# fboehm/DBSLMM

Hardware: AMD Instinct MI355X
Metric: SNPs solved/sec (whole node) + max-|Δβ| vs CPU ref, 1M SNP × 10k indiv (higher is better)
Workload: dtype f64

## Files before the change

### dbslmm_amd/csrc/pcg.hip

```cpp
#include <hip/hip_runtime.h>
#include <stdint.h>

namespace pcg {
constexpr int kT = 128;
constexpr int kRunMax = 8;
constexpr int kMaxNC = 4;
constexpr int kWaves = 4;
constexpr int kVS = kT + 8;
constexpr int kNDot = 5;
constexpr int kQS = 8;
constexpr int kThreads = 256;
constexpr int kFTb = 8;
constexpr int kFRows = kFTb * kT;
constexpr int kFPer = kFRows / kThreads;
constexpr int wave_lds_doubles(int nc) { return 3 * nc * kVS + 4 * nc * 64; }
constexpr size_t lds_bytes(int nc) { return sizeof(double) * kWaves * wave_lds_doubles(nc); }
}

struct PcgBlk {
    int32_t blk, row0, m, ms;
    int32_t ld, Tb, Ns, sco;
    int64_t matoff, vo, po, dof;
    int64_t off16;
    int32_t nc;
    int32_t mshift;
    int32_t fused;
    int32_t pad_;
};

struct PcgArgs {
    const PcgBlk* blk;
    const uint16_t* G16;
    const double* M;
    const int32_t* flags;
    const double* S;
    const double* rsd;
    const double* z;
    const int32_t* slot_out;
    const int32_t* blk_id;
    const double* dshift;
    double *X, *R, *P, *Sv, *W;
    double* U;
    double* part;
    double* dot;
    double* qs;
    int32_t* cnv;
    int32_t* itb;
    int32_t* done;
    int32_t* active;
    int32_t* fin;
    double* beta_s;
    double* beta_l;
    int32_t* status;
    double* mir_s;
    double* mir_l;
    int32_t* mir_st;
    int32_t* mir_flag;
    int32_t run_no;
    int64_t vstride;
    int64_t ns, nl, nbk;
    double tau, rn, c0, tol, inv_sqrt_n;
    int32_t ncopy;
    int32_t run;
    int32_t seed;
};

namespace pcg {

__device__ __forceinline__ void wave_fence() {
    __builtin_amdgcn_fence(__ATOMIC_RELEASE, "wavefront");
    __builtin_amdgcn_wave_barrier();
    __builtin_amdgcn_fence(__ATOMIC_ACQUIRE, "wavefront");
}

template <int Ctrl>
__device__ __forceinline__ double dpp_mov(double v) {
    const uint64_t b = __builtin_bit_cast(uint64_t, v);
    const int lo = __builtin_amdgcn_mov_dpp(static_cast<int>(b & 0xffffffffu), Ctrl, 0xf, 0xf, false);
    const int hi = __builtin_amdgcn_mov_dpp(static_cast<int>(b >> 32), Ctrl, 0xf, 0xf, false);
    return __builtin_bit_cast(double, (static_cast<uint64_t>(static_cast<uint32_t>(hi)) << 32) | static_cast<uint32_t>(lo));
}
template <int X>
__device__ __forceinline__ uint32_t swap_xor(uint32_t x, bool up) {
    if constexpr (X == 16) {
        const auto r = __builtin_amdgcn_permlane16_swap(x, x, false, false);
        return up ? r[0] : r[1];
    } else {
        const auto r = __builtin_amdgcn_permlane32_swap(x, x, false, false);
        return up ? r[0] : r[1];
    }
}
template <int X>
__device__ __forceinline__ double lane_xor(double v) {
#ifndef PCG_NO_DPP
    if constexpr (X == 1) return dpp_mov<0xB1>(v);
    else if constexpr (X == 2) return dpp_mov<0x4E>(v);
    else if constexpr (X == 4) return dpp_mov<0x1B>(dpp_mov<0x141>(v));
    else if constexpr (X == 8) return dpp_mov<0x128>(v);
#ifndef PCG_NO_PERMLANE
    else if constexpr (X == 16 || X == 32) {
        const uint64_t b = __builtin_bit_cast(uint64_t, v);
        const bool up = (__lane_id() & X) != 0;
        const uint32_t lo = swap_xor<X>(static_cast<uint32_t>(b & 0xffffffffu), up);
        const uint32_t hi = swap_xor<X>(static_cast<uint32_t>(b >> 32), up);
        return __builtin_bit_cast(double, (static_cast<uint64_t>(hi) << 32) | lo);
    }
#endif
    else
#endif
        return __shfl_xor(v, X);
}

template <int X2, int X1, int X0>
__device__ __forceinline__ double rscatter8(const double (&v)[8], int lane) {
    const bool h2 = (lane & X2) != 0, h1 = (lane & X1) != 0, h0 = (lane & X0) != 0;
    double u[4], w[2];
#pragma unroll
    for (int q = 0; q < 4; ++q) {
        const double send = h2 ? v[q] : v[q + 4], keep = h2 ? v[q + 4] : v[q];
        u[q] = keep + lane_xor<X2>(send);
    }
#pragma unroll
    for (int q = 0; q < 2; ++q) {
        const double send = h1 ? u[q] : u[q + 2], keep = h1 ? u[q + 2] : u[q];
        w[q] = keep + lane_xor<X1>(send);
    }
    const double send = h0 ? w[0] : w[1], keep = h0 ? w[1] : w[0];
    return keep + lane_xor<X0>(send);
}

__device__ __forceinline__ double wave_sum(double v) {
    v += lane_xor<32>(v);
    v += lane_xor<16>(v);
    v += lane_xor<8>(v);
    v += lane_xor<4>(v);
    v += lane_xor<2>(v);
    v += lane_xor<1>(v);
    return v;
}



__device__ __forceinline__ double ordered_sum(const double* __restrict__ p, int64_t st, int s0, int s1, double acc) {
    for (int s = s0; s < s1; s += 8) {
        double t[8];
#pragma unroll
        for (int u = 0; u < 8; ++u) t[u] = s + u < s1 ? p[static_cast<int64_t>(s + u) * st] : 0.0;
#pragma unroll
        for (int u = 0; u < 8; ++u) acc += t[u];
    }
    return acc;
}

__device__ __forceinline__ bool on_u16(const PcgArgs& a, const PcgBlk& B) {
    return a.G16 != nullptr && (a.flags[B.blk] & 1) == 0;
}

__device__ __forceinline__ double jdiag(const PcgArgs& a, const PcgBlk& B, int i, double dc) {
    return B.mshift ? 1.0 : i < B.ms ? a.c0 + dc : a.c0;
}
__device__ __forceinline__ double col_shift(const PcgArgs& a, const PcgBlk& B, int k) {
    return a.dshift[B.mshift ? a.seed : k];
}

__device__ __forceinline__ void put_beta(const PcgArgs& a, const PcgBlk& B, int i, int k, double x, bool mono) {
    const int so = a.slot_out[B.row0 + i];
    const double bv = mono ? __builtin_nan("") : x * a.inv_sqrt_n;
    if (so >= 0) {
        a.beta_s[k * a.ns + so] = bv;
        if (a.mir_s) a.mir_s[k * a.ns + so] = bv;
    } else {
        a.beta_l[k * a.nl - 1 - so] = bv;
        if (a.mir_l) a.mir_l[k * a.nl - 1 - so] = bv;
    }
}
__device__ __forceinline__ void put_status(const PcgArgs& a, const PcgBlk& B, int k, bool mono) {
    const int st = mono ? DBSLMM_BLOCK_MONOMORPHIC
                        : a.cnv[B.sco + k] == 0 ? DBSLMM_BLOCK_NOT_CONVERGED : DBSLMM_BLOCK_OK;
    const int64_t o = k * a.nbk + a.blk_id[B.blk];
    a.status[o] = st;
    if (a.mir_st) a.mir_st[o] = st;
}

__device__ __forceinline__ double cvt_lo(uint32_t w) {
    double g;
    uint32_t t;
    asm volatile("v_and_b32 %1, 0xffff, %2\n\tv_cvt_f64_u32 %0, %1" : "=v"(g), "=&v"(t) : "v"(w));
    return g;
}
__device__ __forceinline__ double cvt_hi(uint32_t w) {
    double g;
    uint32_t t;
    asm volatile("v_lshrrev_b32 %1, 16, %2\n\tv_cvt_f64_u32 %0, %1" : "=v"(g), "=&v"(t) : "v"(w));
    return g;
}

typedef uint32_t pcg_u4 __attribute__((ext_vector_type(4)));

__device__ __forceinline__ __amdgpu_buffer_rsrc_t g16_rsrc(const uint16_t* base, uint32_t bytes) {
    const uint64_t gb = reinterpret_cast<uint64_t>(base);
    const uint32_t lo = static_cast<uint32_t>(__builtin_amdgcn_readfirstlane(static_cast<int>(gb & 0xffffffffu)));
    const uint32_t hi = static_cast<uint32_t>(__builtin_amdgcn_readfirstlane(static_cast<int>(gb >> 32)));
    const int nb = __builtin_amdgcn_readfirstlane(static_cast<int>(bytes));
    return __builtin_amdgcn_make_buffer_rsrc(reinterpret_cast<void*>((static_cast<uint64_t>(hi) << 32) | lo),
                                             static_cast<short>(0), nb, 0x00020000);
}
constexpr uint32_t kG16Oob = 0x80000000u;

__device__ __forceinline__ void quad_mul16(const pcg_u4 (&raw)[8], bool diagq, int lane, int nc,
                                           const double* vI, const double* vJ, double* rsum, double* csum) {
    const int rg = lane >> 3, cg = lane & 7;
#pragma unroll 1
    for (int k = 0; k < nc; ++k) {
        double vi[8], vj[8], racc[8], cacc[8];
#pragma unroll
        for (int q = 0; q < 8; ++q) {
            vi[q] = vI[k * kVS + 8 * rg + q];
            vj[q] = vJ[k * kVS + 8 * cg + q];
            racc[q] = cacc[q] = 0.0;
        }
        if (!diagq) {
#pragma unroll
            for (int r = 0; r < 8; ++r)
#pragma unroll
                for (int c = 0; c < 8; ++c) {
                    const uint32_t w = raw[r][c >> 1];
                    const double g = (c & 1) ? cvt_hi(w) : cvt_lo(w);
                    racc[r] = __builtin_fma(g, vj[c], racc[r]);
                    cacc[c] = __builtin_fma(g, vi[r], cacc[c]);
                }
        } else {
#pragma unroll
            for (int r = 0; r < 8; ++r)
#pragma unroll
                for (int c = 0; c < 8; ++c) {
                    const uint32_t w = raw[r][c >> 1];
                    const double g = (c & 1) ? cvt_hi(w) : cvt_lo(w);
                    const int dd = 8 * (cg - rg) + c - r;
                    racc[r] = __builtin_fma(dd <= 0 ? g : 0.0, vj[c], racc[r]);
                    cacc[c] = __builtin_fma(dd < 0 ? g : 0.0, vi[r], cacc[c]);
                }
        }
        rsum[k * 64 + lane] += rscatter8<4, 2, 1>(racc, lane);
        csum[k * 64 + lane] += rscatter8<32, 16, 8>(cacc, lane);
    }
}

__device__ __forceinline__ void quad_mul64(const double* __restrict__ base, int64_t ld, int rows_ok, int cols_ok,
                                           bool diagq, int lane, int nc, const double* vI, const double* vJ,
                                           double* rsum, double* csum) {
    const int rg = lane >> 3, cg = lane & 7;
#pragma unroll 1
    for (int k = 0; k < nc; ++k) {
        double vi[8], vj[8], racc[8], cacc[8];
#pragma unroll
        for (int q = 0; q < 8; ++q) {
            vi[q] = vI[k * kVS + 8 * rg + q];
            vj[q] = vJ[k * kVS + 8 * cg + q];
            racc[q] = cacc[q] = 0.0;
        }
#pragma unroll 1
        for (int r = 0; r < 8; ++r)
#pragma unroll
            for (int c = 0; c < 8; ++c) {
                const double g = (r < rows_ok && c < cols_ok) ? base[r * ld + c] : 0.0;
                const int dd = 8 * (cg - rg) + c - r;
                const double gr = !diagq || dd <= 0 ? g : 0.0, gc = !diagq || dd < 0 ? g : 0.0;
#pragma unroll
                for (int q = 0; q < 8; ++q)
                    if (q == r) racc[q] = __builtin_fma(gr, vj[c], racc[q]);
                cacc[c] = __builtin_fma(gc, vi[r], cacc[c]);
            }
        rsum[k * 64 + lane] += rscatter8<4, 2, 1>(racc, lane);
        csum[k * 64 + lane] += rscatter8<32, 16, 8>(cacc, lane);
    }
}

__device__ __forceinline__ void stage_v(const PcgArgs& a, const PcgBlk& B, int T, int nc, int lane, double* v) {
    for (int k = 0; k < nc; ++k) {
        const double* src = a.U + k * a.vstride + B.vo + static_cast<int64_t>(T) * kT;
        const double x0 = src[lane], x1 = src[lane + 64];
        v[k * kVS + lane] = x0;
        v[k * kVS + lane + 64] = x1;
    }
}

__device__ __forceinline__ bool quad_active(const PcgBlk& B, int I, int J, int q) {
    const int qi = q >> 1, qj = q & 1;
    return !(J == I && qj > qi) && I * kT + 64 * qi < B.m && J * kT + 64 * qj < B.m;
}
__device__ __forceinline__ bool next_quad(const PcgBlk& B, int I, int J1, int& J, int& q) {
    for (;;) {
        if (++q == 4) {
            q = 0;
            if (++J > J1) return false;
        }
        if (quad_active(B, I, J, q)) return true;
    }
}

template <bool U16>
__device__ void symv_item(const PcgArgs& a, int4 item, int lane, double* vI, double* vJb, double* rsum,
                          double* csum) {
    const PcgBlk B = a.blk[item.x];
    if (a.done[item.x] || on_u16(a, B) != U16) return;
    const int I = item.y, J0 = item.z, J1 = item.w, nc = B.nc;
    const int64_t ld16 = static_cast<int64_t>(B.Tb) * kT;
    const int rg = lane >> 3, cg = lane & 7;
    auto vj_of = [&](int J) -> double* { return J == I ? vI : vJb + ((J - J0) & 1) * nc * kVS; };
    const __amdgpu_buffer_rsrc_t g16 =
        g16_rsrc(a.G16 + B.off16 + static_cast<int64_t>(I) * kT * ld16, U16 ? static_cast<uint32_t>(kT * ld16 * 2) : 0u);
    auto load = [&](int J, int q, pcg_u4 (&raw)[8], bool none) {
        if constexpr (U16) {
            const int i0 = 64 * (q >> 1) + 8 * rg, j0 = J * kT + 64 * (q & 1) + 8 * cg;
            const bool skip = none || j0 >= B.m || (J == I && (q == 0 || q == 3) && cg > rg);
            const uint32_t o = static_cast<uint32_t>((static_cast<int64_t>(i0) * ld16 + j0) * 2);
#pragma unroll
            for (int r = 0; r < 8; ++r)
                raw[r] = __builtin_amdgcn_raw_buffer_load_b128(
                    g16, (skip || I * kT + i0 + r >= B.m) ? kG16Oob : o + static_cast<uint32_t>(r * ld16 * 2), 0, 0);
        }
    };
    auto mult = [&](int J, int q, const pcg_u4 (&raw)[8]) {
        const int qi = q >> 1, qj = q & 1;
        const bool dq = J == I && qi == qj;
        const double* vj = vj_of(J);
        double* rs = rsum + qi * nc * 64;
        double* cs = csum + qj * nc * 64;
        if constexpr (U16) {
            quad_mul16(raw, dq, lane, nc, vI + 64 * qi, vj + 64 * qj, rs, cs);
        } else {
            const int ib = I * kT + 64 * qi + 8 * rg, jb = J * kT + 64 * qj + 8 * cg;
            quad_mul64(a.M + B.matoff + static_cast<int64_t>(ib) * B.ld + jb, B.ld, B.m - ib, B.m - jb, dq,
                       lane, nc, vI + 64 * qi, vj + 64 * qj, rs, cs);
        }
    };
    auto flush = [&](int J) {
        double* dst = a.part + B.po + (static_cast<int64_t>(J) * B.Ns + I) * nc * kT;
        for (int qj = 0; qj < 2; ++qj)
            for (int k = 0; k < nc; ++k) {
                dst[k * kT + 64 * qj + 8 * cg + rg] = csum[(qj * nc + k) * 64 + lane];
                csum[(qj * nc + k) * 64 + lane] = 0.0;
            }
    };
    pcg_u4 ra[8], rb[8];
    int J = J0, q = 0;
    load(J, q, ra, false);
    stage_v(a, B, I, nc, lane, vI);
    if (J != I) stage_v(a, B, J, nc, lane, vj_of(J));
    for (int t = 0; t < 2 * nc; ++t) rsum[t * 64 + lane] = csum[t * 64 + lane] = 0.0;
    wave_fence();
    auto step = [&](pcg_u4 (&cur)[8], pcg_u4 (&nxt)[8]) -> bool {
        int Jn = J, qn = q;
        const bool more = next_quad(B, I, J1, Jn, qn);
        load(more ? Jn : J, more ? qn : q, nxt, !more);
        if (more && Jn != J && Jn != I) stage_v(a, B, Jn, nc, lane, vj_of(Jn));
        mult(J, q, cur);
        if (!more || Jn != J) flush(J);
        wave_fence();
        J = Jn;
        q = qn;
        return more;
    };
    while (step(ra, rb) && step(rb, ra)) {
    }
    double* dst = a.part + B.po + (static_cast<int64_t>(I) * B.Ns + B.Tb + J0 / a.run) * nc * kT;
    for (int qi = 0; qi < 2; ++qi)
        for (int k = 0; k < nc; ++k) dst[k * kT + 64 * qi + 8 * rg + cg] = rsum[(qi * nc + k) * 64 + lane];
}

}

extern "C" __global__ __launch_bounds__(pcg::kThreads) void dbslmm_pcg_init(PcgArgs a, const int2* __restrict__ rows) {
    using namespace pcg;
    __shared__ double red[kThreads / 64][kMaxNC];
    __shared__ int mono_s;
    const int2 it = rows[blockIdx.x];
    const int bi = it.x, I = it.y, tid = threadIdx.x;
    const PcgBlk B = a.blk[bi];
    const bool u16 = on_u16(a, B);
    const int n = a.ncopy, nc = B.nc;
    if (I == 0) {
        if (tid == 0) mono_s = 0;
        __syncthreads();
        bool mono = false;
        for (int i = tid; i < B.m; i += kThreads) mono |= !(a.rsd[B.row0 + i] < INFINITY);
        if (mono) atomicOr(&mono_s, 1);
        __syncthreads();
        if (tid < n) {
            a.cnv[B.sco + tid] = 0;
            double* q = a.qs + static_cast<int64_t>(B.sco + tid) * kQS;
            q[4] = q[5] = 1.0;
        }
        if (tid == 0) {
            a.itb[bi] = 0;
            a.fin[bi] = 0;
            const bool fz = B.fused && u16;
            a.done[bi] = mono_s ? 2 : fz ? 3 : 0;
            if (!mono_s && !fz) atomicAdd(a.active, 1);
        }
    }
    const int r = tid & (kT - 1), h = tid >> 7, i = I * kT + r;
    const bool in = i < B.m;
    double sv[kMaxNC];
#pragma unroll
    for (int k = 0; k < kMaxNC; ++k) sv[k] = 0.0;
    for (int c = h; c < n; c += 2) {
        const int64_t o = c * a.vstride + B.vo + i;
        const double rhs = in ? a.z[B.row0 + i] : 0.0;
        a.X[o] = 0.0;
        a.P[o] = 0.0;
        if (c < nc) {
            a.Sv[o] = 0.0;
            a.W[o] = 0.0;
            a.R[o] = rhs;
            double uv = 0.0;
            if (in) {
                uv = rhs / jdiag(a, B, i, col_shift(a, B, c));
                if (u16) uv *= a.rsd[B.row0 + i];
            }
            a.U[o] = uv;
        }
    }
#pragma unroll
    for (int k = 0; k < kMaxNC; ++k)
        if (k < nc && (k & 1) == h && in && u16) {
            const double rhs = a.z[B.row0 + i];
            sv[k] = a.S[B.row0 + i] * a.rsd[B.row0 + i] * (rhs / jdiag(a, B, i, col_shift(a, B, k)));
        }
#pragma unroll
    for (int k = 0; k < kMaxNC; ++k) sv[k] = wave_sum(sv[k]);
    if ((tid & 63) == 0)
#pragma unroll
        for (int k = 0; k < kMaxNC; ++k) red[tid >> 6][k] = sv[k];
    __syncthreads();
    if (tid < nc) {
        const int hk = tid & 1;
        a.dot[B.dof + (static_cast<int64_t>(I) * kNDot + 4) * n + tid] = red[2 * hk][tid] + red[2 * hk + 1][tid];
    }
}

template <bool U16>
__device__ __forceinline__ void symv_body(const PcgArgs& a, const int4* __restrict__ items, int32_t n_items) {
    using namespace pcg;
    extern __shared__ double vlds[];
    const int wave = threadIdx.x >> 6, lane = threadIdx.x & 63;
    const int e = blockIdx.x * kWaves + wave;
    if (e >= n_items) return;
    const int nc = a.ncopy;
    double* w = vlds + wave * wave_lds_doubles(nc);
    symv_item<U16>(a, items[e], lane, w, w + nc * kVS, w + 3 * nc * kVS, w + 3 * nc * kVS + 2 * nc * 64);
}
#ifndef PCG_SYMV_WAVES
#define PCG_SYMV_WAVES 2
#endif
extern "C" __global__ __launch_bounds__(pcg::kThreads) __attribute__((amdgpu_waves_per_eu(PCG_SYMV_WAVES, 8)))
void dbslmm_pcg_symv16(PcgArgs a, const int4* __restrict__ items, int32_t n_items) {
    symv_body<true>(a, items, n_items);
}
extern "C" __global__ __launch_bounds__(pcg::kThreads)
void dbslmm_pcg_symv64(PcgArgs a, const int4* __restrict__ items, int32_t n_items) {
    symv_body<false>(a, items, n_items);
}

extern "C" __global__ __launch_bounds__(pcg::kThreads) void dbslmm_pcg_rows(PcgArgs a, const int2* __restrict__ rows) {
    using namespace pcg;
    __shared__ double red[kThreads / 64][kMaxNC][4];
    __shared__ double sig[kMaxNC];
    const int2 it = rows[blockIdx.x];
    const int bi = it.x, I = it.y, tid = threadIdx.x;
    if (a.done[bi]) return;
    const PcgBlk B = a.blk[bi];
    const bool u16 = on_u16(a, B);
    const int n = a.ncopy, nc = B.nc;
    if (tid < nc)
        sig[tid] = ordered_sum(a.dot + B.dof + 4 * n + tid, kNDot * n, 0, B.Tb, 0.0);
    __syncthreads();
    const int r = tid & (kT - 1), h = tid >> 7, i = I * kT + r;
    const bool in = i < B.m;
    const double Si = in ? a.S[B.row0 + i] : 0.0, ri = in ? a.rsd[B.row0 + i] : 0.0;
    const int nrun = (I + a.run) / a.run;
    double dv[kMaxNC][4];
#pragma unroll
    for (int k = 0; k < kMaxNC; ++k)
#pragma unroll
        for (int f = 0; f < 4; ++f) dv[k][f] = 0.0;
#pragma unroll
    for (int k = 0; k < kMaxNC; ++k) {
        if (k >= n || (k & 1) != h) continue;
        const int64_t o = k * a.vstride + B.vo + i;
        if (k < nc) {
            const double* pp = a.part + B.po + static_cast<int64_t>(I) * B.Ns * nc * kT + k * kT + r;
            double y = ordered_sum(pp, nc * kT, I, B.Tb, 0.0);
            y = ordered_sum(pp, nc * kT, B.Tb, B.Tb + nrun, y);
            const double dc = col_shift(a, B, k);
            const double rv = a.R[o];
            const double u = in ? rv / jdiag(a, B, i, dc) : 0.0;
            const double sh = i < B.ms ? dc : 0.0;
            double w = 0.0;
            if (in) {
                if (u16) w = a.tau * a.rn * ri * __builtin_fma(-Si, sig[k] * a.rn, y) + (1.0 - a.tau + sh) * u;
                else w = y + sh * u;
            }
            a.W[o] = w;
            dv[k][0] = rv * u;
            dv[k][1] = w * u;
            dv[k][2] = rv * rv;
        }
        const double xv = a.X[o];
        dv[k][3] = xv * xv;
    }
#pragma unroll
    for (int k = 0; k < kMaxNC; ++k)
#pragma unroll
        for (int f = 0; f < 4; ++f) dv[k][f] = wave_sum(dv[k][f]);
    if ((tid & 63) == 0)
#pragma unroll
        for (int k = 0; k < kMaxNC; ++k)
#pragma unroll
            for (int f = 0; f < 4; ++f) red[tid >> 6][k][f] = dv[k][f];
    __syncthreads();
    if (tid < 4 * n) {
        const int k = tid >> 2, f = tid & 3, hk = k & 1;
        if (f == 3 || k < nc)
            a.dot[B.dof + (static_cast<int64_t>(I) * kNDot + f) * n + k] = red[2 * hk][k][f] + red[2 * hk + 1][k][f];
    }
    if (I == 0 && tid == 0) a.itb[bi] += 1;
}

extern "C" __global__ __launch_bounds__(pcg::kThreads) void dbslmm_pcg_update(PcgArgs a, const int2* __restrict__ rows) {
    using namespace pcg;
    __shared__ double tot[kMaxNC][4];
    __shared__ double coef[kMaxNC][3];
    __shared__ double seedc[2];
    __shared__ int run_s[kMaxNC];
    __shared__ double red[kThreads / 64][kMaxNC];
    const int2 it = rows[blockIdx.x];
    const int bi = it.x, I = it.y, tid = threadIdx.x;
    if (a.done[bi]) return;
    const PcgBlk B = a.blk[bi];
    const bool u16 = on_u16(a, B);
    const int n = a.ncopy, nc = B.nc;
    const int itn = a.itb[bi] - 1;
    const int par = itn & 1;
    if (tid < 4 * n) {
        const int k = tid >> 2, f = tid & 3;
        tot[k][f] = (f == 3 || k < nc) ? ordered_sum(a.dot + B.dof + f * n + k, kNDot * n, 0, B.Tb, 0.0) : 0.0;
    }
    __syncthreads();
    if (B.mshift) {
        if (tid == 0) {
            const double gam = tot[0][0], del = tot[0][1];
            const double* q = a.qs + static_cast<int64_t>(B.sco) * kQS;
            double al, be = 0.0;
            if (itn == 0) {
                al = gam / del;
            } else {
                be = gam / q[2 * par];
                al = gam / (del - be * gam / q[2 * par + 1]);
            }
            seedc[0] = al;
            seedc[1] = be;
        }
        __syncthreads();
        if (tid < n) {
            const int c = tid;
            double* q = a.qs + static_cast<int64_t>(B.sco + c) * kQS;
            const double al = seedc[0], be = seedc[1];
            const double zk = q[4 + 2 * par], zk1 = q[4 + 2 * par + 1];
            const double rr = tot[0][2] * zk * zk, xx = tot[c][3];
            const double t = a.tol * (a.dshift[c] + 1.0 - a.tau);
            const bool conv = a.cnv[B.sco + c] != 0 || rr == 0.0 || rr <= t * t * xx;
            const double e = a.dshift[c] - a.dshift[a.seed];
            const double cp = itn == 0 ? 0.0 : al * be / a.qs[static_cast<int64_t>(B.sco) * kQS + 2 * par + 1];
            const double zn = zk * zk1 / ((1.0 + cp + al * e) * zk1 - cp * zk);
            coef[c][0] = al * zn / zk;
            coef[c][1] = zk1 != 0.0 ? (zk / zk1) * (zk / zk1) * be : 0.0;
            coef[c][2] = zk;
            run_s[c] = conv ? 0 : 1;
            if (I == 0) {
                if (conv && a.cnv[B.sco + c] == 0) a.cnv[B.sco + c] = itn + 1;
                q[4 + 2 * (par ^ 1)] = zn;
                q[4 + 2 * (par ^ 1) + 1] = zk;
            }
        }
        __syncthreads();
        if (I == 0 && tid == 0) {
            double* q = a.qs + static_cast<int64_t>(B.sco) * kQS;
            q[2 * (par ^ 1)] = tot[0][0];
            q[2 * (par ^ 1) + 1] = seedc[0];
        }
    } else {
        if (tid < n) {
            const int k = tid;
            const double gam = tot[k][0], del = tot[k][1], rr = tot[k][2], xx = tot[k][3];
            const double lam = B.ms == B.m ? a.dshift[k] + 1.0 - a.tau : 1.0 - a.tau;
            const double t = a.tol * lam;
            const bool conv = a.cnv[B.sco + k] != 0 || rr == 0.0 || rr <= t * t * xx;
            double al = 0.0, be = 0.0;
            if (!conv) {
                double* q = a.qs + static_cast<int64_t>(B.sco + k) * kQS;
                if (itn == 0) {
                    al = gam / del;
                } else {
                    be = gam / q[2 * par];
                    al = gam / (del - be * gam / q[2 * par + 1]);
                }
                if (I == 0) {
                    q[2 * (par ^ 1)] = gam;
                    q[2 * (par ^ 1) + 1] = al;
                }
            } else if (I == 0 && a.cnv[B.sco + k] == 0) {
                a.cnv[B.sco + k] = itn + 1;
            }
            coef[k][0] = al;
            coef[k][1] = be;
            coef[k][2] = 1.0;
            run_s[k] = conv ? 0 : 1;
        }
        __syncthreads();
    }
    int running = 0;
    for (int k = 0; k < n; ++k) running += run_s[k];
    if (running == 0) {
        const int r = tid & (kT - 1), h = tid >> 7, i = I * kT + r;
        if (i < B.m)
            for (int k = h; k < n; k += 2) put_beta(a, B, i, k, a.X[k * a.vstride + B.vo + i], false);
        if (I == 0 && tid < n) put_status(a, B, tid, false);
        __syncthreads();
        if (tid == 0 &&
            __hip_atomic_fetch_add(a.fin + bi, 1, __ATOMIC_ACQ_REL, __HIP_MEMORY_SCOPE_AGENT) == B.Tb - 1) {
            a.done[bi] = 1;
            atomicSub(a.active, 1);
            if (a.mir_flag)
                for (int c = 0; c < n; ++c)
                    __hip_atomic_store(a.mir_flag + static_cast<int64_t>(bi) * n + c, a.run_no, __ATOMIC_RELEASE,
                                       __HIP_MEMORY_SCOPE_SYSTEM);
        }
        return;
    }
    const int r = tid & (kT - 1), h = tid >> 7, i = I * kT + r;
    const bool in = i < B.m;
    double sv[kMaxNC];
#pragma unroll
    for (int k = 0; k < kMaxNC; ++k) sv[k] = 0.0;
    if (B.mshift) {
        if (in) {
            const int64_t o0 = B.vo + i;
            const double rv = a.R[o0];
#pragma unroll
            for (int c = 0; c < kMaxNC; ++c) {
                if (c >= n || (c & 1) != h || !run_s[c]) continue;
                const int64_t o = c * a.vstride + o0;
                const double p = __builtin_fma(coef[c][1], a.P[o], coef[c][2] * rv);
                a.P[o] = p;
                a.X[o] = __builtin_fma(coef[c][0], p, a.X[o]);
            }
            if (h == 0) {
                const double al = seedc[0], be = seedc[1];
                const double sn = __builtin_fma(be, a.Sv[o0], a.W[o0]);
                const double rn = __builtin_fma(-al, sn, rv);
                a.Sv[o0] = sn;
                a.R[o0] = rn;
                a.U[o0] = u16 ? rn * a.rsd[B.row0 + i] : rn;
                if (u16) sv[0] = a.S[B.row0 + i] * a.rsd[B.row0 + i] * rn;
            }
        }
    } else {
#pragma unroll
        for (int k = 0; k < kMaxNC; ++k) {
            if (k >= n || (k & 1) != h || !run_s[k] || !in) continue;
            const int64_t o = k * a.vstride + B.vo + i;
            const double al = coef[k][0], be = coef[k][1];
            const double dg = jdiag(a, B, i, a.dshift[k]);
            const double u = a.R[o] / dg;
            const double p = __builtin_fma(be, a.P[o], u);
            const double s = __builtin_fma(be, a.Sv[o], a.W[o]);
            const double x = __builtin_fma(al, p, a.X[o]);
            const double rn = __builtin_fma(-al, s, a.R[o]);
            a.P[o] = p;
            a.Sv[o] = s;
            a.X[o] = x;
            a.R[o] = rn;
            a.U[o] = u16 ? (rn / dg) * a.rsd[B.row0 + i] : rn / dg;
            if (u16) sv[k] = a.S[B.row0 + i] * a.rsd[B.row0 + i] * (rn / dg);
        }
    }
#pragma unroll
    for (int k = 0; k < kMaxNC; ++k) sv[k] = wave_sum(sv[k]);
    if ((tid & 63) == 0)
#pragma unroll
        for (int k = 0; k < kMaxNC; ++k) red[tid >> 6][k] = sv[k];
    __syncthreads();
    if (tid < nc && (B.mshift || run_s[tid])) {
        const int hk = tid & 1;
        a.dot[B.dof + (static_cast<int64_t>(I) * kNDot + 4) * n + tid] = red[2 * hk][tid] + red[2 * hk + 1][tid];
    }
}

#ifndef PCG_BLOCK_DEPTH
#define PCG_BLOCK_DEPTH 3
#endif
namespace pcg {
template <int N>
__device__ __forceinline__ void block_sum(double (&v)[N], double* red, int tid) {
#pragma unroll
    for (int k = 0; k < N; ++k) v[k] = wave_sum(v[k]);
    __syncthreads();
    if ((tid & 63) == 0)
#pragma unroll
        for (int k = 0; k < N; ++k) red[(tid >> 6) * N + k] = v[k];
    __syncthreads();
#pragma unroll
    for (int k = 0; k < N; ++k) v[k] = ((red[k] + red[N + k]) + red[2 * N + k]) + red[3 * N + k];
}
constexpr size_t block_lds_bytes(int n) {
    return sizeof(double) * ((5 + 2 * n) * kFRows + 4 * (3 + kMaxNC) + 12 + 3 * kMaxNC + 4);
}
}

__device__ __forceinline__ void pcg_block_solve(const PcgArgs& a, int bi, int cc, int32_t maxit) {
    using namespace pcg;
    extern __shared__ double blds[];
    double* yw = blds;
    double* Ul = blds + 4 * kFRows;
    const int n = a.ncopy;
    double* Xl = Ul + kFRows;
    double* Pl = Xl + n * kFRows;
    double* red = Pl + n * kFRows;
    if (a.done[bi] != 3) return;
    const PcgBlk B = a.blk[bi];
    const int tid = threadIdx.x, lane = tid & 63, wave = tid >> 6;
    const int m = B.m, Tb = B.Tb;
    const bool msh = cc < 0;
    const int nx = msh ? n : 1;
    const double dc = msh ? col_shift(a, B, 0) : a.dshift[cc];
    double r[kFPer], sv[kFPer], wv[kFPer], Sr[kFPer], Rr[kFPer], sg[1] = {0.0};
#pragma unroll
    for (int q = 0; q < kFPer; ++q) {
        const int i = tid + kThreads * q;
        const bool in = i < m;
        r[q] = in ? a.z[B.row0 + i] : 0.0;
        Sr[q] = in ? a.S[B.row0 + i] : 0.0;
        Rr[q] = in ? a.rsd[B.row0 + i] : 0.0;
        sv[q] = wv[q] = 0.0;
        double u = 0.0;
        if (in) {
            u = (r[q] / jdiag(a, B, i, dc)) * Rr[q];
            sg[0] += Sr[q] * u;
        }
        Ul[i] = u;
        for (int w = 0; w < 4; ++w) yw[w * kFRows + i] = 0.0;
        for (int c = 0; c < nx; ++c) Xl[c * kFRows + i] = Pl[c * kFRows + i] = 0.0;
    }
    block_sum(sg, red, tid);
    double sig = sg[0];
    const int Q = (m + 63) / 64;
    const int nq = Q * (Q + 1) / 2;
    const int64_t ld16 = static_cast<int64_t>(Tb) * kT;
    const int rg = lane >> 3, cg = lane & 7;
    auto quad_of = [&](int t, int& qi, int& qj) {
        qi = static_cast<int>((sqrtf(8.0f * t + 1.0f) - 1.0f) * 0.5f);
        while (qi * (qi + 1) / 2 > t) --qi;
        while ((qi + 1) * (qi + 2) / 2 <= t) ++qi;
        qj = t - qi * (qi + 1) / 2;
    };
    const __amdgpu_buffer_rsrc_t g16 = g16_rsrc(a.G16 + B.off16, static_cast<uint32_t>(ld16 * ld16 * 2));
    auto load = [&](int t, pcg_u4 (&raw)[8]) {
        int qi, qj;
        quad_of(t, qi, qj);
        const int r0 = 64 * qi + 8 * rg, c0 = 64 * qj + 8 * cg;
        const bool skip = t >= nq || c0 >= m || (qi == qj && cg > rg);
        const uint32_t o = static_cast<uint32_t>((r0 * static_cast<int>(ld16) + c0) * 2);
#pragma unroll
        for (int rr = 0; rr < 8; ++rr)
            raw[rr] = __builtin_amdgcn_raw_buffer_load_b128(
                g16, (skip || r0 + rr >= m) ? kG16Oob : o + static_cast<uint32_t>(rr * ld16 * 2), 0, 0);
    };
    auto mult = [&](int t, const pcg_u4 (&raw)[8]) {
        int qi, qj;
        quad_of(t, qi, qj);
        const bool dq = qi == qj;
        double vi[8], vj[8], racc[8], cacc[8];
#pragma unroll
        for (int q = 0; q < 8; ++q) {
            vi[q] = Ul[64 * qi + 8 * rg + q];
            vj[q] = Ul[64 * qj + 8 * cg + q];
            racc[q] = cacc[q] = 0.0;
        }
        if (!dq) {
#pragma unroll
            for (int rr = 0; rr < 8; ++rr)
#pragma unroll
                for (int c = 0; c < 8; ++c) {
                    const uint32_t w = raw[rr][c >> 1];
                    const double g = (c & 1) ? cvt_hi(w) : cvt_lo(w);
                    racc[rr] = __builtin_fma(g, vj[c], racc[rr]);
                    cacc[c] = __builtin_fma(g, vi[rr], cacc[c]);
                }
        } else {
#pragma unroll
            for (int rr = 0; rr < 8; ++rr)
#pragma unroll
                for (int c = 0; c < 8; ++c) {
                    const uint32_t w = raw[rr][c >> 1];
                    const double g = (c & 1) ? cvt_hi(w) : cvt_lo(w);
                    const int dd = 8 * (cg - rg) + c - rr;
                    racc[rr] = __builtin_fma(dd <= 0 ? g : 0.0, vj[c], racc[rr]);
                    cacc[c] = __builtin_fma(dd < 0 ? g : 0.0, vi[rr], cacc[c]);
                }
        }
        double* y = yw + wave * kFRows;
        const int ri = 64 * qi + 8 * rg + cg, ci = 64 * qj + 8 * cg + rg;
        y[ri] += rscatter8<4, 2, 1>(racc, lane);
        wave_fence();
        y[ci] += rscatter8<32, 16, 8>(cacc, lane);
    };
    double* st = red + 4 * (3 + kMaxNC);
    int* flag = reinterpret_cast<int*>(st + 12 + 3 * kMaxNC);
    if (tid == 0) {
        for (int c = 0; c < kMaxNC; ++c) {
            st[4 + c] = st[8 + c] = 1.0;
            flag[c] = c >= n;
        }
    }
    int it = 0;
    for (; it < maxit; ++it) {
        __syncthreads();
        {
#if PCG_BLOCK_DEPTH == 3
            pcg_u4 ra[8], rb[8], rc[8];
            int t = wave;
            load(t, ra);
            load(t + 4, rb);
            while (t < nq) {
                load(t + 8, rc);
                mult(t, ra);
                t += 4;
                if (t >= nq) break;
                load(t + 8, ra);
                mult(t, rb);
                t += 4;
                if (t >= nq) break;
                load(t + 8, rb);
                mult(t, rc);
                t += 4;
            }
#else
            pcg_u4 ra[8], rb[8];
            int t = wave;
            load(t, ra);
            while (t < nq) {
                load(t + 4, rb);
                mult(t, ra);
                t += 4;
                if (t >= nq) break;
                load(t + 4, ra);
                mult(t, rb);
                t += 4;
            }
#endif
        }
        __syncthreads();
        double d[3 + kMaxNC];
#pragma unroll
        for (int k = 0; k < 3 + kMaxNC; ++k) d[k] = 0.0;
#pragma unroll
        for (int q = 0; q < kFPer; ++q) {
            const int i = tid + kThreads * q;
            double y = 0.0;
            if (i < Tb * kT) {
                y = ((yw[i] + yw[kFRows + i]) + yw[2 * kFRows + i]) + yw[3 * kFRows + i];
#pragma unroll
                for (int w = 0; w < 4; ++w) yw[w * kFRows + i] = 0.0;
            }
            if (i < m) {
                const double Si = Sr[q], ri = Rr[q];
                const double u = r[q] / jdiag(a, B, i, dc);
                const double sh = i < B.ms ? dc : 0.0;
                const double w = a.tau * a.rn * ri * __builtin_fma(-Si, sig * a.rn, y) + (1.0 - a.tau + sh) * u;
                wv[q] = w;
                d[0] += r[q] * u;
                d[1] += w * u;
                d[2] += r[q] * r[q];
                for (int c = 0; c < nx; ++c) {
                    const double xv = Xl[c * kFRows + i];
                    d[3 + c] += xv * xv;
                }
            }
        }
        block_sum(d, red, tid);
        if (tid == 0) {
            const double gam = d[0], del = d[1], rr = d[2];
            double al, be = 0.0;
            if (it == 0) {
                al = gam / del;
            } else {
                be = gam / st[0];
                al = gam / (del - be * gam / st[1]);
            }
            int running = 0;
            if (msh) {
                const double cp = it == 0 ? 0.0 : al * be / st[1];
                for (int c = 0; c < n; ++c) {
                    const double zk = st[4 + c], zk1 = st[8 + c];
                    const double t = a.tol * (a.dshift[c] + 1.0 - a.tau);
                    const double rrc = rr * zk * zk;
                    if (!flag[c] && (rrc == 0.0 || rrc <= t * t * d[3 + c])) {
                        flag[c] = 1;
                        a.cnv[B.sco + c] = it + 1;
                    }
                    const double e = a.dshift[c] - a.dshift[a.seed];
                    const double zn = zk * zk1 / ((1.0 + cp + al * e) * zk1 - cp * zk);
                    st[12 + 3 * c] = al * zn / zk;
                    st[12 + 3 * c + 1] = zk1 != 0.0 ? (zk / zk1) * (zk / zk1) * be : 0.0;
                    st[12 + 3 * c + 2] = zk;
                    st[8 + c] = zk;
                    st[4 + c] = zn;
                    running += flag[c] ? 0 : 1;
                }
            } else {
                const double lam = B.ms == B.m ? dc + 1.0 - a.tau : 1.0 - a.tau;
                const double t = a.tol * lam;
                if (rr == 0.0 || rr <= t * t * d[3]) {
                    flag[0] = 1;
                    a.cnv[B.sco + cc] = it + 1;
                }
                running = flag[0] ? 0 : 1;
            }
            st[0] = gam;
            st[1] = al;
            st[2] = al;
            st[3] = be;
            flag[kMaxNC] = running;
        }
        __syncthreads();
        if (flag[kMaxNC] == 0) break;
        const double al = st[2], be = st[3];
        double sg2[1] = {0.0};
#pragma unroll
        for (int q = 0; q < kFPer; ++q) {
            const int i = tid + kThreads * q;
            if (i >= m) continue;
            const double rsd_i = Rr[q];
            double rn;
            if (msh) {
                for (int c = 0; c < n; ++c) {
                    if (flag[c]) continue;
                    const int o = c * kFRows + i;
                    const double pv = __builtin_fma(st[12 + 3 * c + 1], Pl[o], st[12 + 3 * c + 2] * r[q]);
                    Pl[o] = pv;
                    Xl[o] = __builtin_fma(st[12 + 3 * c], pv, Xl[o]);
                }
                const double sn = __builtin_fma(be, sv[q], wv[q]);
                rn = __builtin_fma(-al, sn, r[q]);
                sv[q] = sn;
                r[q] = rn;
                Ul[i] = rn * rsd_i;
            } else {
                const double dg = jdiag(a, B, i, dc);
                const double u = r[q] / dg;
                const double pv = __builtin_fma(be, Pl[i], u);
                const double sn = __builtin_fma(be, sv[q], wv[q]);
                Pl[i] = pv;
                Xl[i] = __builtin_fma(al, pv, Xl[i]);
                rn = __builtin_fma(-al, sn, r[q]);
                sv[q] = sn;
                r[q] = rn;
                Ul[i] = (rn / dg) * rsd_i;
            }
            sg2[0] += Sr[q] * Ul[i];
        }
        block_sum(sg2, red, tid);
        sig = sg2[0];
    }
#pragma unroll
    for (int q = 0; q < kFPer; ++q) {
        const int i = tid + kThreads * q;
        if (i < m)
            for (int c = 0; c < nx; ++c) put_beta(a, B, i, msh ? c : cc, Xl[c * kFRows + i], false);
    }
    if (tid == 0) {
        atomicMax(a.itb + bi, it + (it < maxit ? 1 : 0));
        for (int c = 0; c < nx; ++c) put_status(a, B, msh ? c : cc, false);
    }
    if (a.mir_flag) {
        __syncthreads();
        if (tid == 0)
            for (int c = 0; c < nx; ++c)
                __hip_atomic_store(a.mir_flag + static_cast<int64_t>(bi) * n + (msh ? c : cc), a.run_no,
                                   __ATOMIC_RELEASE, __HIP_MEMORY_SCOPE_SYSTEM);
    }
}

extern "C" __global__ __launch_bounds__(pcg::kThreads)
#if PCG_BLOCK_DEPTH == 3
__attribute__((amdgpu_waves_per_eu(1, 8), amdgpu_num_vgpr(312)))
#else
__attribute__((amdgpu_waves_per_eu(2, 8)))
#endif
void dbslmm_pcg_block(PcgArgs a, const int2* __restrict__ list, int32_t n_list, int32_t* __restrict__ next,
                      int32_t maxit) {
    __shared__ int e_s;
    for (;;) {
        __syncthreads();
        if (threadIdx.x == 0) e_s = atomicAdd(next, 1);
        __syncthreads();
        const int e = e_s;
        if (e >= n_list) break;
        pcg_block_solve(a, list[e].x, list[e].y, maxit);
    }
}

extern "C" __global__ __launch_bounds__(pcg::kThreads) void dbslmm_pcg_final(PcgArgs a, const int2* __restrict__ rows) {
    using namespace pcg;
    const int2 it = rows[blockIdx.x];
    const int bi = it.x, I = it.y, tid = threadIdx.x;
    const int done = a.done[bi];
    if (done == 3 || done == 1) return;
    const PcgBlk B = a.blk[bi];
    const bool mono = done == 2;
    const int r = tid & (kT - 1), h = tid >> 7, i = I * kT + r;
    if (i < B.m)
        for (int k = h; k < a.ncopy; k += 2) put_beta(a, B, i, k, a.X[k * a.vstride + B.vo + i], mono);
    if (I == 0 && tid < a.ncopy) put_status(a, B, tid, mono);
}
```

Measured before the change: 156.5 million.

## Hoist global loads ahead of reductions and widen ordered-sum batches in PCG kernels

The rows and update kernels now issue their per-element loads (R, X, P, Sv, W, S, rsd, partial sums) up front, before the barrier and the cross-tile dot reductions, so load latency overlaps the serial reductions. Lanes at the end of the block now compute the sigma reduction instead of the first lanes. The ordered_sum helper moves to a shared header with a templated batch width of 16 instead of 8, and the partial-sum loop is merged into one call. The block solve preloads slot_out and block id and takes status from a local convergence flag instead of re-reading global memory. The cost is higher register pressure, plus reliance on a `flag` variable that must exist in the elided code.

New measurement: 158.9 million, median of 4. 1.02x the previous value.

```diff
diff --git a/dbslmm_amd/csrc/ordered_sum.hpp b/dbslmm_amd/csrc/ordered_sum.hpp
--- /dev/null
+++ b/dbslmm_amd/csrc/ordered_sum.hpp
@@ -0,0 +1,26 @@
+#pragma once
+#include <stdint.h>
+
+#if defined(__HIPCC__)
+#define ORDERED_SUM_FN __attribute__((host)) __attribute__((device)) inline __attribute__((always_inline))
+#else
+#define ORDERED_SUM_FN inline
+#endif
+#if defined(__clang__)
+#define ORDERED_SUM_UNROLL _Pragma("unroll")
+#else
+#define ORDERED_SUM_UNROLL
+#endif
+
+template <int B = 32>
+ORDERED_SUM_FN double ordered_sum(const double* __restrict__ p, int64_t st, int s0, int s1, double acc) {
+    static_assert(B > 0, "batch width");
+    for (int s = s0; s < s1; s += B) {
+        double t[B];
+        ORDERED_SUM_UNROLL
+        for (int u = 0; u < B; ++u) t[u] = s + u < s1 ? p[static_cast<int64_t>(s + u) * st] : 0.0;
+        ORDERED_SUM_UNROLL
+        for (int u = 0; u < B; ++u) acc += t[u];
+    }
+    return acc;
+}
diff --git a/dbslmm_amd/csrc/pcg.hip b/dbslmm_amd/csrc/pcg.hip
--- a/dbslmm_amd/csrc/pcg.hip
+++ b/dbslmm_amd/csrc/pcg.hip
@@ -1,5 +1,7 @@
 #include <hip/hip_runtime.h>
 #include <stdint.h>
+
+#include "ordered_sum.hpp"
 
 namespace pcg {
 constexpr int kT = 128;
@@ -10,6 +12,7 @@
 constexpr int kNDot = 5;
 constexpr int kQS = 8;
 constexpr int kThreads = 256;
+constexpr int kSumBatch = 16;
 constexpr int kFTb = 8;
 constexpr int kFRows = kFTb * kT;
 constexpr int kFPer = kFRows / kThreads;
@@ -139,19 +142,6 @@
     return v;
 }
 
-
-
-__device__ __forceinline__ double ordered_sum(const double* __restrict__ p, int64_t st, int s0, int s1, double acc) {
-    for (int s = s0; s < s1; s += 8) {
-        double t[8];
-#pragma unroll
-        for (int u = 0; u < 8; ++u) t[u] = s + u < s1 ? p[static_cast<int64_t>(s + u) * st] : 0.0;
-#pragma unroll
-        for (int u = 0; u < 8; ++u) acc += t[u];
-    }
-    return acc;
-}
-
 __device__ __forceinline__ bool on_u16(const PcgArgs& a, const PcgBlk& B) {
     return a.G16 != nullptr && (a.flags[B.blk] & 1) == 0;
 }
@@ -163,8 +153,7 @@
     return a.dshift[B.mshift ? a.seed : k];
 }
 
-__device__ __forceinline__ void put_beta(const PcgArgs& a, const PcgBlk& B, int i, int k, double x, bool mono) {
-    const int so = a.slot_out[B.row0 + i];
+__device__ __forceinline__ void put_beta_at(const PcgArgs& a, int so, int k, double x, bool mono) {
     const double bv = mono ? __builtin_nan("") : x * a.inv_sqrt_n;
     if (so >= 0) {
         a.beta_s[k * a.ns + so] = bv;
@@ -174,12 +163,18 @@
         if (a.mir_l) a.mir_l[k * a.nl - 1 - so] = bv;
     }
 }
-__device__ __forceinline__ void put_status(const PcgArgs& a, const PcgBlk& B, int k, bool mono) {
-    const int st = mono ? DBSLMM_BLOCK_MONOMORPHIC
-                        : a.cnv[B.sco + k] == 0 ? DBSLMM_BLOCK_NOT_CONVERGED : DBSLMM_BLOCK_OK;
-    const int64_t o = k * a.nbk + a.blk_id[B.blk];
+__device__ __forceinline__ void put_beta(const PcgArgs& a, const PcgBlk& B, int i, int k, double x, bool mono) {
+    put_beta_at(a, a.slot_out[B.row0 + i], k, x, mono);
+}
+__device__ __forceinline__ void put_status_as(const PcgArgs& a, int id, int k, int st) {
+    const int64_t o = k * a.nbk + id;
     a.status[o] = st;
     if (a.mir_st) a.mir_st[o] = st;
+}
+__device__ __forceinline__ void put_status(const PcgArgs& a, const PcgBlk& B, int k, bool mono) {
+    put_status_as(a, a.blk_id[B.blk], k,
+                  mono ? DBSLMM_BLOCK_MONOMORPHIC
+                       : a.cnv[B.sco + k] == 0 ? DBSLMM_BLOCK_NOT_CONVERGED : DBSLMM_BLOCK_OK);
 }
 
 __device__ __forceinline__ double cvt_lo(uint32_t w) {
@@ -469,17 +464,33 @@
     __shared__ double sig[kMaxNC];
     const int2 it = rows[blockIdx.x];
     const int bi = it.x, I = it.y, tid = threadIdx.x;
-    if (a.done[bi]) return;
+    const int dn = a.done[bi];
     const PcgBlk B = a.blk[bi];
+    if (dn) return;
     const bool u16 = on_u16(a, B);
     const int n = a.ncopy, nc = B.nc;
-    if (tid < nc)
-        sig[tid] = ordered_sum(a.dot + B.dof + 4 * n + tid, kNDot * n, 0, B.Tb, 0.0);
-    __syncthreads();
     const int r = tid & (kT - 1), h = tid >> 7, i = I * kT + r;
     const bool in = i < B.m;
     const double Si = in ? a.S[B.row0 + i] : 0.0, ri = in ? a.rsd[B.row0 + i] : 0.0;
+    double rv[kMaxNC], xv[kMaxNC], y[kMaxNC];
+#pragma unroll
+    for (int k = 0; k < kMaxNC; ++k) {
+        rv[k] = xv[k] = y[k] = 0.0;
+        if (k >= n || (k & 1) != h) continue;
+        const int64_t o = k * a.vstride + B.vo + i;
+        if (k < nc) rv[k] = a.R[o];
+        xv[k] = a.X[o];
+    }
+    const int ks = tid - (kThreads - kMaxNC);
+    if (ks >= 0 && ks < nc) sig[ks] = ordered_sum<kSumBatch>(a.dot + B.dof + 4 * n + ks, kNDot * n, 0, B.Tb, 0.0);
     const int nrun = (I + a.run) / a.run;
+#pragma unroll
+    for (int k = 0; k < kMaxNC; ++k) {
+        if (k >= nc || (k & 1) != h) continue;
+        const double* pp = a.part + B.po + static_cast<int64_t>(I) * B.Ns * nc * kT + k * kT + r;
+        y[k] = ordered_sum<kSumBatch>(pp, nc * kT, I, B.Tb + nrun, 0.0);
+    }
+    __syncthreads();
     double dv[kMaxNC][4];
 #pragma unroll
     for (int k = 0; k < kMaxNC; ++k)
@@ -490,25 +501,20 @@
         if (k >= n || (k & 1) != h) continue;
         const int64_t o = k * a.vstride + B.vo + i;
         if (k < nc) {
-            const double* pp = a.part + B.po + static_cast<int64_t>(I) * B.Ns * nc * kT + k * kT + r;
-            double y = ordered_sum(pp, nc * kT, I, B.Tb, 0.0);
-            y = ordered_sum(pp, nc * kT, B.Tb, B.Tb + nrun, y);
             const double dc = col_shift(a, B, k);
-            const double rv = a.R[o];
-            const double u = in ? rv / jdiag(a, B, i, dc) : 0.0;
+            const double u = in ? rv[k] / jdiag(a, B, i, dc) : 0.0;
             const double sh = i < B.ms ? dc : 0.0;
             double w = 0.0;
             if (in) {
-                if (u16) w = a.tau * a.rn * ri * __builtin_fma(-Si, sig[k] * a.rn, y) + (1.0 - a.tau + sh) * u;
-                else w = y + sh * u;
+                if (u16) w = a.tau * a.rn * ri * __builtin_fma(-Si, sig[k] * a.rn, y[k]) + (1.0 - a.tau + sh) * u;
+                else w = y[k] + sh * u;
             }
             a.W[o] = w;
-            dv[k][0] = rv * u;
+            dv[k][0] = rv[k] * u;
             dv[k][1] = w * u;
-            dv[k][2] = rv * rv;
-        }
-        const double xv = a.X[o];
-        dv[k][3] = xv * xv;
+            dv[k][2] = rv[k] * rv[k];
+        }
+        dv[k][3] = xv[k] * xv[k];
     }
 #pragma unroll
     for (int k = 0; k < kMaxNC; ++k)
@@ -537,15 +543,41 @@
     __shared__ double red[kThreads / 64][kMaxNC];
     const int2 it = rows[blockIdx.x];
     const int bi = it.x, I = it.y, tid = threadIdx.x;
-    if (a.done[bi]) return;
+    const int dn = a.done[bi];
     const PcgBlk B = a.blk[bi];
+    const int itn = a.itb[bi] - 1;
+    if (dn) return;
     const bool u16 = on_u16(a, B);
     const int n = a.ncopy, nc = B.nc;
-    const int itn = a.itb[bi] - 1;
     const int par = itn & 1;
+    const int r = tid & (kT - 1), h = tid >> 7, i = I * kT + r;
+    const bool in = i < B.m;
+    const double Sdi = in ? a.S[B.row0 + i] : 0.0, rsdi = in ? a.rsd[B.row0 + i] : 0.0;
+    double vX[2], vP[2], vR[2], vS[2], vW[2];
+#pragma unroll
+    for (int j = 0; j < 2; ++j) {
+        const int k = h + 2 * j;
+        vX[j] = vP[j] = vR[j] = vS[j] = vW[j] = 0.0;
+        if (k >= n) continue;
+        const int64_t o = k * a.vstride + B.vo + i;
+        vX[j] = a.X[o];
+        vP[j] = a.P[o];
+        if (!B.mshift) {
+            vR[j] = a.R[o];
+            vS[j] = a.Sv[o];
+            vW[j] = a.W[o];
+        }
+    }
+    if (B.mshift) {
+        vR[0] = a.R[B.vo + i];
+        if (h == 0) {
+            vS[0] = a.Sv[B.vo + i];
+            vW[0] = a.W[B.vo + i];
+        }
+    }
     if (tid < 4 * n) {
         const int k = tid >> 2, f = tid & 3;
-        tot[k][f] = (f == 3 || k < nc) ? ordered_sum(a.dot + B.dof + f * n + k, kNDot * n, 0, B.Tb, 0.0) : 0.0;
+        tot[k][f] = (f == 3 || k < nc) ? ordered_sum<kSumBatch>(a.dot + B.dof + f * n + k, kNDot * n, 0, B.Tb, 0.0) : 0.0;
     }
     __syncthreads();
     if (B.mshift) {
@@ -623,9 +655,10 @@
     int running = 0;
     for (int k = 0; k < n; ++k) running += run_s[k];
     if (running == 0) {
-        const int r = tid & (kT - 1), h = tid >> 7, i = I * kT + r;
-        if (i < B.m)
-            for (int k = h; k < n; k += 2) put_beta(a, B, i, k, a.X[k * a.vstride + B.vo + i], false);
+        if (in)
+#pragma unroll
+            for (int j = 0; j < 2; ++j)
+                if (h + 2 * j < n) put_beta(a, B, i, h + 2 * j, vX[j], false);
         if (I == 0 && tid < n) put_status(a, B, tid, false);
         __syncthreads();
         if (tid == 0 &&
@@ -639,31 +672,29 @@
         }
         return;
     }
-    const int r = tid & (kT - 1), h = tid >> 7, i = I * kT + r;
-    const bool in = i < B.m;
     double sv[kMaxNC];
 #pragma unroll
     for (int k = 0; k < kMaxNC; ++k) sv[k] = 0.0;
     if (B.mshift) {
         if (in) {
             const int64_t o0 = B.vo + i;
-            const double rv = a.R[o0];
+            const double rv = vR[0];
 #pragma unroll
             for (int c = 0; c < kMaxNC; ++c) {
                 if (c >= n || (c & 1) != h || !run_s[c]) continue;
                 const int64_t o = c * a.vstride + o0;
-                const double p = __builtin_fma(coef[c][1], a.P[o], coef[c][2] * rv);
+                const double p = __builtin_fma(coef[c][1], vP[c >> 1], coef[c][2] * rv);
                 a.P[o] = p;
-                a.X[o] = __builtin_fma(coef[c][0], p, a.X[o]);
+                a.X[o] = __builtin_fma(coef[c][0], p, vX[c >> 1]);
             }
             if (h == 0) {
                 const double al = seedc[0], be = seedc[1];
-                const double sn = __builtin_fma(be, a.Sv[o0], a.W[o0]);
+                const double sn = __builtin_fma(be, vS[0], vW[0]);
                 const double rn = __builtin_fma(-al, sn, rv);
                 a.Sv[o0] = sn;
                 a.R[o0] = rn;
-                a.U[o0] = u16 ? rn * a.rsd[B.row0 + i] : rn;
-                if (u16) sv[0] = a.S[B.row0 + i] * a.rsd[B.row0 + i] * rn;
+                a.U[o0] = u16 ? rn * rsdi : rn;
+                if (u16) sv[0] = Sdi * rsdi * rn;
             }
         }
     } else {
@@ -673,17 +704,18 @@
             const int64_t o = k * a.vstride + B.vo + i;
             const double al = coef[k][0], be = coef[k][1];
             const double dg = jdiag(a, B, i, a.dshift[k]);
-            const double u = a.R[o] / dg;
-            const double p = __builtin_fma(be, a.P[o], u);
-            const double s = __builtin_fma(be, a.Sv[o], a.W[o]);
-            const double x = __builtin_fma(al, p, a.X[o]);
-            const double rn = __builtin_fma(-al, s, a.R[o]);
+            const int j = k >> 1;
+            const double u = vR[j] / dg;
+            const double p = __builtin_fma(be, vP[j], u);
+            const double s = __builtin_fma(be, vS[j], vW[j]);
+            const double x = __builtin_fma(al, p, vX[j]);
+            const double rn = __builtin_fma(-al, s, vR[j]);
             a.P[o] = p;
             a.Sv[o] = s;
             a.X[o] = x;
             a.R[o] = rn;
-            a.U[o] = u16 ? (rn / dg) * a.rsd[B.row0 + i] : rn / dg;
-            if (u16) sv[k] = a.S[B.row0 + i] * a.rsd[B.row0 + i] * (rn / dg);
+            a.U[o] = u16 ? (rn / dg) * rsdi : rn / dg;
+            if (u16) sv[k] = Sdi * rsdi * (rn / dg);
         }
     }
 #pragma unroll
@@ -736,10 +768,13 @@
     const int nx = msh ? n : 1;
     const double dc = msh ? col_shift(a, B, 0) : a.dshift[cc];
     double r[kFPer], sv[kFPer], wv[kFPer], Sr[kFPer], Rr[kFPer], sg[1] = {0.0};
+    int so[kFPer];
+    const int bid = a.blk_id[B.blk];
 #pragma unroll
     for (int q = 0; q < kFPer; ++q) {
         const int i = tid + kThreads * q;
         const bool in = i < m;
+        so[q] = in ? a.slot_out[B.row0 + i] : 0;
         r[q] = in ? a.z[B.row0 + i] : 0.0;
         Sr[q] = in ? a.S[B.row0 + i] : 0.0;
         Rr[q] = in ? a.rsd[B.row0 + i] : 0.0;
@@ -978,11 +1013,12 @@
     for (int q = 0; q < kFPer; ++q) {
         const int i = tid + kThreads * q;
         if (i < m)
-            for (int c = 0; c < nx; ++c) put_beta(a, B, i, msh ? c : cc, Xl[c * kFRows + i], false);
+            for (int c = 0; c < nx; ++c) put_beta_at(a, so[q], msh ? c : cc, Xl[c * kFRows + i], false);
     }
     if (tid == 0) {
         atomicMax(a.itb + bi, it + (it < maxit ? 1 : 0));
-        for (int c = 0; c < nx; ++c) put_status(a, B, msh ? c : cc, false);
+        for (int c = 0; c < nx; ++c)
+            put_status_as(a, bid, msh ? c : cc, flag[c] ? DBSLMM_BLOCK_OK : DBSLMM_BLOCK_NOT_CONVERGED);
     }
     if (a.mir_flag) {
         __syncthreads();
```
